# celo-org/celo-bls-snark-rs

Hardware: AMD Instinct MI355X
Metric: BLS12-377 G1 MSM scalar-muls/sec (higher is better)
Workload: dtype u32 limbs (28-bit radix, 64-bit column accumulators); 1 GPU; BLS12-377 G1 Pippenger MSM, 2^20 random bases/scalars per GPU, inputs resident in HBM; bases_per_gpu=1048576, window_bits=16, windows=16, buckets=524288

## Files before the change

celo-bls-snark-rs_amd/csrc/msm_engine.h:

```cpp
#pragma once

namespace celo {

extern "C" int celo_ifma_available();
extern "C" int celo_ifma_horner_377(const uint64_t* pts, size_t stride, const int32_t* order, int steps, uint64_t* out, int* inf);
extern "C" int celo_ifma_horner_761(const uint64_t* pts, size_t stride, const int32_t* order, int steps, uint64_t* out, int* inf);
typedef int (*ifma_horner_fn)(const uint64_t*, size_t, const int32_t*, int, uint64_t*, int*);
template <class F> struct IfmaHorner { static constexpr ifma_horner_fn fn = nullptr; };
template <> struct IfmaHorner<Fp<P377>> { static constexpr ifma_horner_fn fn = &celo_ifma_horner_377; };
template <> struct IfmaHorner<Fp<P761>> { static constexpr ifma_horner_fn fn = &celo_ifma_horner_761; };

struct MsmTimings {
  float convert = 0, sort = 0, accumulate = 0, reduce = 0, total = 0;
};

}
#include "msm_ba.h"
namespace celo {
template <> struct BaCfg<G_761> { static constexpr bool enabled = true; };

struct MsmTuning {
  bool narrow_windows, use_glv, use_gls, gls_force, lane_bitsum, host_threads, seg_occupancy, side_convert, side_convert_all, fx_compact;
  uint32_t seg_min, seg_min_shard, bitsum_lanes_max_shard;
  int seg_halves;
// ... 77 lines not shown
  bool host_threads = MsmTuning::get().host_threads;
  bool lane_horner = true;
  bool lane_bitsum = MsmTuning::get().lane_bitsum;
  uint32_t BITSUM_LANES_MAX = MsmTuning::get().bitsum_lanes_max;

  struct Plan { bool glv; uint32_t n; int sbits, c, nw, kn; };
  Plan plan(size_t n_) const {
    Plan p;
    p.glv = GlvExpand<G>::AVAILABLE && big_subgroup_points && use_glv && n_ >= (size_t(1) << 14);
    p.n = p.glv ? 2u * (uint32_t)n_ : (uint32_t)n_;
    p.sbits = p.glv ? GlvExpand<G>::BITS : G::SCALAR_BITS;
    p.c = force_c ? force_c : (p.glv ? window_bits_glv(p.n) : window_bits(p.n));
    p.nw = (p.sbits + p.c) / p.c;
    p.kn = narrow_top(p.c) ? p.nw * p.c - (p.sbits + 1) : 0;
    return p;
  }
  static int window_bit(const Plan& p, int w) {
    const int wide = p.nw - p.kn;
    return w < wide ? w * p.c : wide * p.c + (w - wide) * (p.c - 1);
  }
  int run_device(const uint64_t* d_ark_bases, const uint8_t* d_inf, const uint32_t* d_scalars, size_t n_, uint64_t* out_jac,
                 hipStream_t stream) {
    return run_device_windows(d_ark_bases, d_inf, d_scalars, n_, 0, 0, out_jac, nullptr, stream);
  }
  struct HostIn { const uint64_t* bases; const uint8_t* inf; const uint64_t* scalars; uint32_t chunks, head_split, tail_split; bool ark_zero; };
  static constexpr uint32_t HOST_HEAD_SPLIT_DEFAULT = 1, HOST_TAIL_SPLIT_DEFAULT = 0;
  int run_device_windows(const uint64_t* d_ark_bases, const uint8_t* d_inf, const uint32_t* d_scalars, size_t n_, int win_lo, int win_cnt,
                         uint64_t* out_jac, uint64_t* out_xyzz, hipStream_t stream, const FixedTable* fx = nullptr, const HostIn* hin = nullptr) {
    if (n_ == 0) {
      if (out_jac) write_identity(out_jac);
      if (out_xyzz) memset(out_xyzz, 0, 4 * IO::ARK64 * 8);
      return 0;
    }
    if (n_ >= (size_t(1) << 30)) return 2;
    if (fx && (win_cnt || n_ > fx->n || fx->cf < 16 || fx->cf > 22)) return 2;
    Plan pl = plan(n_);
    uint32_t fx_Ep = 0;
    uint8_t* d_fx_v8 = nullptr; uint16_t* d_fx_dg = nullptr; uint32_t* d_fx_cnt = nullptr;
    if (fx && fx->NV > 2 && fx->NV <= 128 && !win_cnt && n_ <= fx->n && fx->cf >= 16 && fx->cf <= 22 && MsmTuning::get().fx_compact) {
      const size_t E = fx->E();
      const size_t o_dg = (E + 255) & ~size_t(255), o_cnt = o_dg + ((E * 2 + 255) & ~size_t(255)), need = o_cnt + 256 * 4;
      if (need > fxs_bytes) {
        if (fxs) (void)hipFree(fxs);
        fxs = nullptr; fxs_bytes = 0;
        HIP_TRY(hipMalloc((void**)&fxs, need + need / 8), 1);
        fxs_bytes = need + need / 8;
      }
      d_fx_v8 = fxs; d_fx_dg = (uint16_t*)(fxs + o_dg); d_fx_cnt = (uint32_t*)(fxs + o_cnt);
      HIP_TRY(hipMemsetAsync(d_fx_cnt, 0, 256 * 4, stream), 1);
      hipLaunchKernelGGL((k_fixed_digits_c<SW, G::SCALAR_BITS>), dim3((fx->n + 255) / 256), dim3(256), 0, stream, d_scalars, fx->tinf, d_fx_v8, d_fx_dg, d_fx_cnt, fx->n,
                         (uint32_t)n_, fx->cf, fx->W, fx->NV, fx->M);
      uint32_t h_cnt[128];
      HIP_TRY(hipMemcpyAsync(h_cnt, d_fx_cnt, fx->NV * 4, hipMemcpyDeviceToHost, stream), 1);
      HIP_TRY(hipStreamSynchronize(stream), 1);
      uint32_t mx = 0;
      for (uint32_t v = 0; v < fx->NV; v++) mx = h_cnt[v] > mx ? h_cnt[v] : mx;
      const uint64_t ep = ((uint64_t)mx + 4095) & ~uint64_t(4095);
      if (ep >= 4096 && ep * 2 <= E) fx_Ep = (uint32_t)ep;
    }
    if (fx) { pl.glv = false; pl.n = fx_Ep ? fx_Ep : fx->E(); pl.sbits = G::SCALAR_BITS; pl.c = 16; pl.nw = (int)fx->NV; pl.kn = 0; }
    if (hin && (fx || pl.glv || win_cnt || hin->chunks < 1 || hin->chunks > 64 || !side_stream_.get() || !sort_stream_.get())) return 2;
    const bool glv = pl.glv;
    const uint32_t n = pl.n;
    const int sbits = pl.sbits, c = pl.c, nw_all = pl.nw;
    if (win_cnt < 0 || win_lo < 0 || (win_cnt && win_lo + win_cnt > nw_all)) return 2;
    const int w0 = win_cnt ? win_lo : 0;
    const int nw = win_cnt ? win_cnt : nw_all;
    if ((uint64_t)n * (uint64_t)nw_all >= (uint64_t(1) << 32)) return 2;
    const uint32_t B = 1u << (c - 1);
    const uint32_t total = (uint32_t)nw * B;
    uint32_t K = 0, cm = n;
    uint32_t clen[HOST_CHUNKS_MAX];
    if (hin) K = host_chunk_plan(n, hin->chunks, hin->head_split, hin->tail_split, cm, clen);
    const uint32_t ns = hin ? cm : n, nws = hin ? K * (uint32_t)nw : (uint32_t)nw, vw = hin ? (uint32_t)nw : 0u;
    const uint32_t npad = hin ? K * cm : n;
    if ((uint64_t)npad * (uint64_t)nw_all >= (uint64_t(1) << 32)) return 2;
    const uint32_t total_s = nws * B;
    const int seg_h = MsmTuning::get().seg_halves ? MsmTuning::get().seg_halves : (glv ? 3 : 4);
    uint32_t SEG = (uint32_t)seg_h * ((fx && !fx_Ep ? n / (uint32_t)nw_all : ns) / B + 1) / 2;
    uint32_t seg_min = MsmTuning::get().seg_min;
    if (win_cnt && MsmTuning::get().seg_occupancy) {
      const uint64_t adds = (uint64_t)n * (uint64_t)nw;
      const uint32_t lanes = (sizeof(F) <= 14 * sizeof(uint32_t)) ? 131072u : 65536u;
      const uint32_t occ = (uint32_t)((adds + lanes - 1) / lanes);
      if (occ < SEG) { SEG = occ; seg_min = MsmTuning::get().seg_min_shard; }
    }
    if (fx && !MsmTuning::get().seg_halves) {
      const uint32_t lanes = (sizeof(F) <= 14 * sizeof(uint32_t)) ? 131072u : 65536u;
      const uint32_t occ = fx->E() / (lanes * 8u) + 1u;
      if (occ < SEG) SEG = occ;
    }
    if (SEG < seg_min) SEG = seg_min;
    if (SEG > SIZE_BINS - 1) SEG = SIZE_BINS - 1;
    const uint32_t PW = B + ns / SEG + 1;
    const uint32_t slots = nws * PW;
    const int LB = c - 1;
    const uint32_t res_pts = (uint32_t)(LB + 1) * (uint32_t)nw;
    const uint32_t half_pts = (uint32_t)nw * (B / 2 + B / 4);

    size_t off = 0;
    auto take = [&](size_t bytes) { size_t o = off; off += (bytes + 255) & ~size_t(255); return o; };
    const size_t o_bases = take(fx ? 0 : (size_t)npad * IO::AFF_WORDS * 4);
    const size_t o_sc2 = take(glv ? (size_t)n * 16 : 0);
    const size_t o_digits = take((size_t)npad * nw_all * 2);
    const size_t o_remap = take(fx_Ep ? (size_t)n * nw_all * 4 : 0);
    const size_t o_sorted = take((size_t)ns * nws * 4);
    const uint32_t HIB = LB < 8 ? 0u : (uint32_t)LB - 8u, NBIN = 1u << HIB;
    uint32_t KB2 = ns / (64 * NBIN > 4096 ? 64 * NBIN : 4096);
    if (KB2 < 1) KB2 = 1;
    if (KB2 > 64) KB2 = 64;
    const uint32_t chunk2 = (ns + KB2 - 1) / KB2;
    const size_t o_blockcnt = take((size_t)nws * NBIN * KB2 * 4);
    const size_t o_binstart = take((size_t)nws * (NBIN + 1) * 4);
    const size_t o_tileprefix = take((size_t)nws * (NBIN + 1) * 4);
    const size_t o_recidx = take((size_t)ns * nws * 4);
    const size_t o_reckey = take((size_t)ns * nws);
    const size_t o_counts = take((size_t)total_s * 4);
    const size_t o_starts = take((size_t)total_s * 4);
    const size_t o_piecesof = take((size_t)total_s * 4);
    const size_t o_plen = take((size_t)slots * 4);
    constexpr size_t BINS_STRIDE = SIZE_BINS + 64;
    const size_t o_bins = take(BINS_STRIDE * 4 * (hin ? K : 1u));
    const size_t o_zero_end = off;
    const size_t o_pfirst = take((size_t)total_s * 4);
    const size_t o_big = take((size_t)total_s * 4);
    const size_t o_mid = take((size_t)total_s * 4);
    const size_t o_pbucket = take(hin ? (size_t)slots * 4 : 0);
    const size_t o_carrier = take(hin ? (size_t)total * IO::XYZZ_WORDS * 4 : 0);
    const size_t o_pstart = take((size_t)slots * 4);
    const size_t o_order = take((size_t)slots * 4);
    const size_t o_partials = take((size_t)slots * IO::XYZZ_WORDS * 4);
    const size_t o_work = take(((size_t)res_pts + 2 * (size_t)half_pts + 64) * IO::XYZZ_WORDS * 4);
    const int ba_ovr = batched_affine_override().load();
    const bool use_ba = BaCfg<G>::enabled && !hin && !fx && (ba_ovr >= 0 ? ba_ovr != 0 : MsmTuning::get().batched_affine != 0) && ns / B >= 8;
    const int ba_occ = MsmTuning::get().ba_occ;
    uint32_t ba_lanes = use_ba ? BA_LANES_OCC1 * (uint32_t)ba_occ * MsmTuning::get().ba_rounds : 0;
    if (use_ba && ba_lanes > (slots + 255) / 256 * 256) ba_lanes = (slots + 255) / 256 * 256;
    const uint32_t ba_pref_slots = use_ba ? ((slots + ba_lanes - 1) / ba_lanes) * (SEG / 2) : 0;
    const size_t o_ba_pts = take(use_ba ? (size_t)ns * nws * IO::AFF_WORDS * 4 : 0);
    const size_t o_ba_pref = take(use_ba ? (size_t)ba_pref_slots * ba_lanes * F::WORDS * 4 : 0);
    if (ensure(off)) return 1;
    if (res_pts > H_OUT_POINTS) return 2;
    char* A = arena;
    uint32_t* d_bases = fx ? fx->table : (uint32_t*)(A + o_bases);
    uint16_t* d_digits_all = (uint16_t*)(A + o_digits);
    uint16_t* d_digits = d_digits_all + (size_t)w0 * n;
    uint32_t* d_sorted = (uint32_t*)(A + o_sorted);
    uint32_t* d_blockcnt = (uint32_t*)(A + o_blockcnt);
    uint32_t* d_binstart = (uint32_t*)(A + o_binstart);
    uint32_t* d_recidx = (uint32_t*)(A + o_recidx);
    uint8_t* d_reckey = (uint8_t*)(A + o_reckey);
    uint32_t* d_tileprefix = (uint32_t*)(A + o_tileprefix);
    uint32_t* d_counts = (uint32_t*)(A + o_counts);
    uint32_t* d_starts = (uint32_t*)(A + o_starts);
    uint32_t* d_pfirst = (uint32_t*)(A + o_pfirst);
    uint32_t* d_piecesof = (uint32_t*)(A + o_piecesof);
    uint32_t* d_big = (uint32_t*)(A + o_big);
    uint32_t* d_mid = (uint32_t*)(A + o_mid);
    uint32_t* d_pstart = (uint32_t*)(A + o_pstart);
    uint32_t* d_plen = (uint32_t*)(A + o_plen);
    uint32_t* d_order = (uint32_t*)(A + o_order);
    uint32_t* d_bins = (uint32_t*)(A + o_bins);
    uint32_t* d_nwork = d_bins + SIZE_BINS;
    uint32_t* d_nbig = d_bins + SIZE_BINS + 1;
    uint32_t* d_nmid = d_bins + SIZE_BINS + 2;
    uint32_t* d_partials = (uint32_t*)(A + o_partials);
    uint32_t* d_work = (uint32_t*)(A + o_work);

    uint32_t* d_pbucket = hin ? (uint32_t*)(A + o_pbucket) : nullptr;
    uint32_t* d_carrier = hin ? (uint32_t*)(A + o_carrier) : nullptr;
    HIP_TRY(hipEventRecord(ev[0], stream), 1);
    const uint32_t region = ns / NBIN;
    const uint32_t ts_threads = region <= 2048 ? 256u : region <= 4096 ? 512u : 1024u;
    const uint32_t TILE = TILE_EPT * ts_threads, max_tiles = NBIN + ns / TILE + 1;
    uint32_t* d_remap = fx_Ep ? (uint32_t*)(A + o_remap) : nullptr;
    auto sort_windows = [&](uint32_t wb, uint32_t wn, hipStream_t st) {
      hipLaunchKernelGGL((k_part_hist<G>), dim3(KB2, wn), dim3(1024), 0, st, d_digits, d_blockcnt, ns, chunk2, NBIN, wb);
      hipLaunchKernelGGL((k_part_scan<G>), dim3(wn), dim3(1024), 0, st, d_blockcnt, d_binstart, d_tileprefix, NBIN, KB2, TILE, wb);
      hipLaunchKernelGGL((k_part_scatter<G>), dim3(KB2, wn), dim3(1024), 0, st, d_digits, d_blockcnt, d_recidx, d_reckey, ns, chunk2, HIB, NBIN, (const uint32_t*)d_remap, vw, wb);
      hipLaunchKernelGGL((k_tile_count<G>), dim3(max_tiles, wn), dim3(ts_threads), 0, st, d_reckey, d_binstart, d_tileprefix, d_counts, ns, B, HIB, NBIN, wb);
      hipLaunchKernelGGL((k_tile_sort<G>), dim3(max_tiles, wn), dim3(ts_threads), 0, st, d_recidx, d_reckey, d_binstart, d_tileprefix, d_counts,
                         d_starts, d_sorted, d_pfirst, d_pstart, d_plen, d_big, d_nbig, d_mid, d_nmid, ns, B, HIB, NBIN, SEG, PW, d_pbucket, vw, wb);
    };
    if (hin) {
      hipStream_t cs = side_stream_.get(), ss = sort_stream_.get();
      struct Drain { hipStream_t a, b, c; bool armed; ~Drain() { if (armed) { (void)hipStreamSynchronize(a); (void)hipStreamSynchronize(b); (void)hipStreamSynchronize(c); } } } drain{cs, ss, stream, true};
      if (ev_copy.size() < 3 * (size_t)K + 1) {
        const size_t have = ev_copy.size();
        ev_copy.resize(3 * (size_t)K + 1, nullptr);
        for (size_t i = have; i < ev_copy.size(); i++) HIP_TRY(hipEventCreateWithFlags(&ev_copy[i], hipEventDisableTiming), 1);
      }
      hipEvent_t* ev_sc = ev_copy.data();
      hipEvent_t* ev_bs = ev_copy.data() + K;
      hipEvent_t* ev_so = ev_copy.data() + 2 * K;
      HIP_TRY(hipMemsetAsync(d_counts, 0, o_zero_end - o_counts, stream), 1);
      HIP_TRY(hipMemsetAsync(d_carrier, 0, (size_t)total * IO::XYZZ_WORDS * 4, stream), 1);
      HIP_TRY(hipEventRecord(ev_copy[3 * K], stream), 1);
      HIP_TRY(hipStreamWaitEvent(ss, ev_copy[3 * K], 0), 1);
      constexpr size_t PT_BYTES = 2 * (size_t)IO::ARK64 * 8;
      const uint32_t cslots = (uint32_t)nw * PW;
      ArkCoord<IO::ARK64> ark_one;
      F::one().to_ark(ark_one.v);
      if (hin->ark_zero && d_inf != d_in_inf) return 2;
      size_t hlo = 0;
      for (uint32_t k = 0; k < K; hlo += clen[k], k++) {
        const size_t lo = (size_t)k * cm, cnt = clen[k];
        if (hin->ark_zero) {
          HIP_TRY(hipMemcpyAsync((char*)d_ark_bases + lo * PT_BYTES, (const char*)hin->bases + hlo * PT_BYTES, cnt * PT_BYTES, hipMemcpyHostToDevice, cs), 1);
          HIP_TRY(hipEventRecord(ev_bs[k], cs), 1);
        }
        HIP_TRY(hipMemcpyAsync((char*)d_scalars + lo * SW * 4, (const char*)hin->scalars + hlo * SW * 4, cnt * SW * 4, hipMemcpyHostToDevice, cs), 1);
        if (hin->inf) HIP_TRY(hipMemcpyAsync((char*)d_inf + lo, hin->inf + hlo, cnt, hipMemcpyHostToDevice, cs), 1);
        HIP_TRY(hipEventRecord(ev_sc[k], cs), 1);
        HIP_TRY(hipStreamWaitEvent(ss, ev_sc[k], 0), 1);
        if (hin->ark_zero) {
          HIP_TRY(hipStreamWaitEvent(ss, ev_bs[k], 0), 1);
          hipLaunchKernelGGL((k_flag_ark_zero<G>), dim3((unsigned)((cnt + 255) / 256)), dim3(256), 0, ss, d_ark_bases + lo * 2 * IO::ARK64,
                             hin->inf ? d_inf + lo : nullptr, d_in_inf + lo, cnt, ark_one);
        }
        if (launch_digits<SW, G::SCALAR_BITS>(c, d_scalars, d_inf, d_digits_all, (uint32_t)(lo + cnt), ss, cm, (k + 1) * cm, k * cm)) return 3;
        sort_windows(k * (uint32_t)nw, (uint32_t)nw, ss);
        uint32_t* bins_k = d_bins + (size_t)k * BINS_STRIDE;
        hipLaunchKernelGGL((k_size_hist<G>), dim3(cslots / 256 < 512 ? (cslots + 255) / 256 : 512), dim3(256), 0, ss, d_plen + (size_t)k * cslots, bins_k, cslots);
        hipLaunchKernelGGL((k_size_scan<G>), dim3(1), dim3(1024), 0, ss, bins_k, bins_k + SIZE_BINS);
        hipLaunchKernelGGL((k_size_scatter<G>), dim3((cslots + 4095) / 4096), dim3(1024), 0, ss, d_plen + (size_t)k * cslots, bins_k, d_order + (size_t)k * cslots, cslots);
        HIP_TRY(hipEventRecord(ev_so[k], ss), 1);
        if (k == 0) {
          HIP_TRY(hipStreamWaitEvent(stream, ev_so[0], 0), 1);
          HIP_TRY(hipEventRecord(ev[1], stream), 1);
          HIP_TRY(hipEventRecord(ev[2], stream), 1);
        }
        if (!hin->ark_zero) {
          HIP_TRY(hipMemcpyAsync((char*)d_ark_bases + lo * PT_BYTES, (const char*)hin->bases + hlo * PT_BYTES, cnt * PT_BYTES, hipMemcpyHostToDevice, cs), 1);
          HIP_TRY(hipEventRecord(ev_bs[k], cs), 1);
        }
        HIP_TRY(hipStreamWaitEvent(stream, ev_bs[k], 0), 1);
        if (k) HIP_TRY(hipStreamWaitEvent(stream, ev_so[k], 0), 1);
        hipLaunchKernelGGL((k_convert_bases<G>), dim3((unsigned)((cnt + 255) / 256)), dim3(256), 0, stream, d_ark_bases + lo * 2 * IO::ARK64, d_bases + lo * IO::AFF_WORDS, cnt);
        hipLaunchKernelGGL((k_accumulate_chunk<G>), dim3((cslots + 255) / 256), dim3(256), 0, stream, d_bases, d_sorted, d_pstart + (size_t)k * cslots, d_plen + (size_t)k * cslots,
                           d_order + (size_t)k * cslots, bins_k + SIZE_BINS, d_partials + (size_t)k * cslots * IO::XYZZ_WORDS, d_pbucket + (size_t)k * cslots, d_carrier, k ? 1u : 0u);
      }
      drain.armed = false;
    } else {
    const bool side = (win_cnt || MsmTuning::get().side_convert_all) && !glv && MsmTuning::get().side_convert && side_stream_.get() && ev_side[0];
    if (fx) {
    } else if (side) {
      HIP_TRY(hipEventRecord(ev_side[0], stream), 1);
      HIP_TRY(hipStreamWaitEvent(side_stream_.get(), ev_side[0], 0), 1);
      hipLaunchKernelGGL((k_convert_bases<G>), dim3((n + 255) / 256), dim3(256), 0, side_stream_.get(), d_ark_bases, d_bases, (size_t)n);
      HIP_TRY(hipEventRecord(ev_side[1], side_stream_.get()), 1);
    } else if (glv) GlvExpand<G>::launch(d_ark_bases, d_inf, d_scalars, (uint32_t)n_, d_bases, (uint32_t*)(A + o_sc2), stream);
    else hipLaunchKernelGGL((k_convert_bases<G>), dim3((n + 255) / 256), dim3(256), 0, stream, d_ark_bases, d_bases, (size_t)n);
    HIP_TRY(hipEventRecord(ev[1], stream), 1);
    if (fx && fx_Ep) {
      HIP_TRY(hipMemsetAsync(d_digits_all, 0xFF, (size_t)n * nw_all * 2, stream), 1);
      HIP_TRY(hipMemsetAsync(d_fx_cnt + 128, 0, 128 * 4, stream), 1);
      const uint32_t E32 = (uint32_t)fx->E();
      hipLaunchKernelGGL((k_fixed_place<G>), dim3((E32 + 1023) / 1024 < 4096 ? (E32 + 1023) / 1024 : 4096), dim3(1024), 0, stream, d_fx_v8, d_fx_dg, d_fx_cnt + 128, d_digits_all,
                         d_remap, E32, n, fx->NV);
    } else if (fx) hipLaunchKernelGGL((k_fixed_digits<SW, G::SCALAR_BITS>), dim3((fx->n + 255) / 256), dim3(256), 0, stream, d_scalars, fx->tinf, d_digits_all, fx->n, (uint32_t)n_,
                               fx->cf, fx->W, fx->NV, fx->M);
    else if (glv) { if (launch_digits<4, GlvExpand<G>::BITS>(c, (const uint32_t*)(A + o_sc2), nullptr, d_digits_all, n, stream)) return 3; }
    else if (launch_digits<SW, G::SCALAR_BITS>(c, d_scalars, d_inf, d_digits_all, n, stream)) return 3;
    HIP_TRY(hipMemsetAsync(d_counts, 0, o_zero_end - o_counts, stream), 1);
    sort_windows(0, (uint32_t)nw, stream);
    hipLaunchKernelGGL((k_size_hist<G>), dim3(slots / 256 < 512 ? (slots + 255) / 256 : 512), dim3(256), 0, stream, d_plen, d_bins, slots);
    hipLaunchKernelGGL((k_size_scan<G>), dim3(1), dim3(1024), 0, stream, d_bins, d_nwork);
    hipLaunchKernelGGL((k_size_scatter<G>), dim3((slots + 4095) / 4096), dim3(1024), 0, stream, d_plen, d_bins, d_order, slots);
    if (side) HIP_TRY(hipStreamWaitEvent(stream, ev_side[1], 0), 1);
    HIP_TRY(hipEventRecord(ev[2], stream), 1);
    if constexpr (BaCfg<G>::enabled) if (use_ba) {
      uint32_t* d_ba_pts = (uint32_t*)(A + o_ba_pts);
      const int levels = MsmTuning::get().ba_levels;
      if (ba_occ == 2)
        hipLaunchKernelGGL((k_ba_levels<G, 2>), dim3(ba_lanes / 256), dim3(256), 0, stream, d_bases, d_sorted, d_pstart, d_plen, d_order, d_nwork, d_ba_pts,
                           (uint32_t*)(A + o_ba_pref), ba_lanes, levels, ba_pref_slots);
      else
        hipLaunchKernelGGL((k_ba_levels<G, 1>), dim3(ba_lanes / 256), dim3(256), 0, stream, d_bases, d_sorted, d_pstart, d_plen, d_order, d_nwork, d_ba_pts,
                           (uint32_t*)(A + o_ba_pref), ba_lanes, levels, ba_pref_slots);
      hipLaunchKernelGGL((k_accumulate_ba<G>), dim3((slots + 255) / 256), dim3(256), 0, stream, d_ba_pts, d_pstart, d_plen, d_order, d_nwork, d_partials, levels);
    }
    if (!use_ba) launch_accumulate<G>(slots, stream, d_bases, d_sorted, d_pstart, d_plen, d_order, d_nwork, d_partials);
    }
    HIP_TRY(hipEventRecord(ev[3], stream), 1);
    const uint32_t mid_blocks = win_cnt ? (total + 20) / 21 < 16384 ? (total + 20) / 21 : 16384 : 1024;
    const uint32_t cfirst = hin ? 1u : 0u;
    if (lane_bitsum) hipLaunchKernelGGL((k_combine_mid_lanes<G>), dim3(mid_blocks), dim3(64), 0, stream, d_mid, d_nmid, d_counts, d_pfirst, d_partials, d_piecesof, SEG, cfirst);
    else hipLaunchKernelGGL((k_combine_mid<G>), dim3(256), dim3(128), 0, stream, d_mid, d_nmid, d_counts, d_pfirst, d_partials, d_piecesof, SEG, cfirst);
    hipLaunchKernelGGL((k_combine_big<G>), dim3(256), dim3(256), 0, stream, d_big, d_nbig, d_counts, d_pfirst, d_partials, d_piecesof, SEG, cfirst);
    const uint32_t* d_leaf = d_partials;
    const uint32_t* d_leaf_counts = d_counts;
    if (hin) {
      hipLaunchKernelGGL((k_merge_carried<G>), dim3((total + 127) / 128), dim3(128), 0, stream, d_counts, d_pfirst, d_partials, d_carrier, total, K, SEG);
      d_leaf = d_carrier; d_leaf_counts = nullptr;
    }
    {
      struct Arr { uint32_t at, per_window; bool born; int level; };
      uint32_t half_at[2] = {res_pts, res_pts + half_pts};
      Arr tree = {0, B, true, LB};
      std::vector<Arr> lists;
      for (int t = 1; t <= LB; t++) {
        BitsumJobs jobs;
        jobs.njobs = 0;
        uint32_t cursor = half_at[t & 1], total_out = 0;
        auto push = [&](uint32_t src, uint32_t outs_per_window, uint32_t mode, int result_slot) -> uint32_t {
          const uint32_t outs = outs_per_window * (uint32_t)nw;
          uint32_t dst;
          if (result_slot >= 0) dst = (uint32_t)result_slot * (uint32_t)nw;
          else { dst = cursor; cursor += outs; }
          const int j = (int)jobs.njobs++;
          total_out += outs;
          jobs.end[j] = total_out; jobs.src[j] = src; jobs.dst[j] = dst; jobs.mode[j] = mode;
          return dst;
        };
        std::vector<Arr> next_lists;
        if (tree.level >= 2) {
          const uint32_t outs = tree.per_window / 4;
          const uint32_t dst = push(tree.at, outs, tree.level == LB ? 3u : 1u, outs == 1 ? tree.level : -1);
          if (outs > 1) next_lists.push_back({dst, outs, false, tree.level});
        } else {
          push(tree.at, 1, 4u, 1);
        }
        for (const Arr& L : lists) {
          const uint32_t outs = L.per_window / 2;
          const uint32_t dst = push(L.at, outs, 0u, outs == 1 ? L.level : -1);
          if (outs > 1) next_lists.push_back({dst, outs, false, L.level});
        }
        {
          const uint32_t outs = tree.per_window / 2;
          const uint32_t dst = push(tree.at, outs, tree.level == LB ? 2u : 0u, outs == 1 ? 0 : -1);
          tree = {dst, outs, true, tree.level - 1};
        }
        lists.swap(next_lists);
        if (lane_bitsum && total_out <= (win_cnt ? MsmTuning::get().bitsum_lanes_max_shard : BITSUM_LANES_MAX))
          hipLaunchKernelGGL((k_bitsum_lanes<G>), dim3((total_out + 20) / 21), dim3(64), 0, stream, d_leaf, d_leaf_counts, d_pfirst, d_piecesof, SEG, d_work, jobs);
        else
          hipLaunchKernelGGL((k_bitsum<G>), dim3((total_out + 127) / 128), dim3(128), 0, stream, d_leaf, d_leaf_counts, d_pfirst, d_piecesof, SEG,
                             d_work, jobs);
      }
      hipLaunchKernelGGL((k_results_to_ark<G>), dim3((4 * res_pts + 63) / 64), dim3(64), 0, stream, d_work, res_pts);
    }
    HIP_TRY(hipEventRecord(ev[4], stream), 1);
    HIP_TRY(hipMemcpyAsync(h_out, d_work, (size_t)res_pts * IO::XYZZ_WORDS * 4, hipMemcpyDeviceToHost, stream), 1);
    HIP_TRY(hipEventRecord(ev[5], stream), 1);
    HIP_TRY(hipStreamSynchronize(stream), 1);
    HIP_TRY(hipGetLastError(), 1);
    (void)hipEventElapsedTime(&tm.convert, ev[0], ev[1]);
    (void)hipEventElapsedTime(&tm.sort, ev[1], ev[2]);
    (void)hipEventElapsedTime(&tm.accumulate, ev[2], ev[3]);
    (void)hipEventElapsedTime(&tm.reduce, ev[3], ev[4]);
    (void)hipEventElapsedTime(&tm.total, ev[0], ev[5]);
    last_c = c; last_nw = nw; last_buckets = total; last_glv = glv;
    typedef typename HostField<F>::type HF;
    const uint64_t* h64 = reinterpret_cast<const uint64_t*>(h_out);
    constexpr size_t PT64 = (size_t)IO::XYZZ_WORDS / 2;
    horner_steps.clear();
    const int kn = pl.kn;
    (void)sbits;
    if (fx) {
      int top = LB - 1;
      while (((uint64_t)(nw - 1) * fx->M) >> (top + 1)) top++;
      for (int t = top; t >= 0; t--) {
        horner_steps.push_back(-1);
        for (int v = 0; v < nw; v++) if ((((uint64_t)v * fx->M) >> t) & 1) horner_steps.push_back(v | HORNER_NODBL);
        if (t <= LB - 1) for (int v = 0; v < nw; v++) horner_steps.push_back(((LB - t) * nw + v) | HORNER_NODBL);
      }
      for (int v = 0; v < nw; v++) horner_steps.push_back(v | HORNER_NODBL);
    } else
    for (int w = nw - 1; w >= 0; w--) {
      horner_steps.push_back(-1);
      for (int l = (w0 + w >= nw_all - kn ? 2 : 1); l <= LB; l++) horner_steps.push_back(l * nw + w);
      horner_steps.push_back(w | HORNER_NODBL);
    }
    auto run_list = [&](const int32_t* steps, int count) {
      if (IfmaHorner<F>::fn && celo_ifma_available()) {
        uint64_t r[4 * IO::ARK64];
        int inf = 0;
        if (IfmaHorner<F>::fn(h64, PT64, steps, count, r, &inf) == 0) return inf ? HXyzz<HF>::identity() : HXyzz<HF>::load(r, IO::ARK64);
      }
      return host64_horner<HF>(h64, PT64, IO::ARK64, steps, count);
    };
    constexpr int HT = (sizeof(HF) > 6 * 8) ? HOST_HORNER_THREADS : 1;
    HXyzz<HF> total_pt;
    if (HT > 1 && host_threads && (fx ? horner_steps.size() >= 64 : nw >= 2 * HT)) {
      int start[HT + 1], dbls[HT];
      if (fx) {
        int adds_total = 0;
        for (int k = 0; k < (int)horner_steps.size(); k++) adds_total += horner_steps[k] >= 0 ? 1 : 0;
        int g = 0, adds = 0;
        start[0] = 0;
        for (int k = 0; k < (int)horner_steps.size(); k++) {
          if (horner_steps[k] < 0 && g + 1 < HT && k > start[g] && adds * HT >= (g + 1) * adds_total) start[++g] = k;
          adds += horner_steps[k] >= 0 ? 1 : 0;
        }
        while (g + 1 < HT) start[++g] = (int)horner_steps.size();
        start[HT] = (int)horner_steps.size();
        for (int j = 0; j < HT; j++) {
          dbls[j] = 0;
          for (int k = start[j]; k < start[j + 1]; k++) if (horner_steps[k] < 0 || !(horner_steps[k] & HORNER_NODBL)) dbls[j]++;
        }
      } else {
        int wdone = 0, g = 0;
        start[0] = 0;
        for (int k = 0; k < (int)horner_steps.size(); k++) {
          if (horner_steps[k] >= 0 && (horner_steps[k] & HORNER_NODBL)) {
            wdone++;
            if (wdone == (g + 1) * nw / HT && g + 1 < HT) start[++g] = k + 1;
          }
        }
        start[HT] = (int)horner_steps.size();
        for (int j = 0; j < HT; j++) {
          dbls[j] = 0;
          for (int k = start[j]; k < start[j + 1]; k++) if (horner_steps[k] < 0 || !(horner_steps[k] & HORNER_NODBL)) dbls[j]++;
        }
      }
      HXyzz<HF> part[HT];
      std::thread th[HT - 1];
      bool started[HT - 1];
      for (int j = 1; j < HT; j++) {
        started[j - 1] = true;
        try { th[j - 1] = std::thread([&, j] { part[j] = run_list(horner_steps.data() + start[j], start[j + 1] - start[j]); }); }
        catch (const std::system_error&) { started[j - 1] = false; }
      }
      part[0] = run_list(horner_steps.data() + start[0], start[1] - start[0]);
      for (int j = 1; j < HT; j++) {
        if (started[j - 1]) th[j - 1].join();
        else part[j] = run_list(horner_steps.data() + start[j], start[j + 1] - start[j]);
      }
      total_pt = part[0];
      for (int j = 1; j < HT; j++) {
        for (int d = 0; d < dbls[j]; d++) total_pt = hxyzz_dbl(total_pt);
        hxyzz_add(total_pt, part[j]);
      }
    } else {
      total_pt = run_list(horner_steps.data(), (int)horner_steps.size());
    }
    if (out_xyzz) {
      if (total_pt.is_identity()) memset(out_xyzz, 0, 4 * IO::ARK64 * 8);
      else { total_pt.X.store(out_xyzz); total_pt.Y.store(out_xyzz + IO::ARK64); total_pt.ZZ.store(out_xyzz + 2 * IO::ARK64); total_pt.ZZZ.store(out_xyzz + 3 * IO::ARK64); }
    }
    if (out_jac) write_host_jacobian(total_pt, out_jac);
    return 0;
  }
  typedef typename HostField<F>::type HostF;
  static void write_host_jacobian(const HXyzz<HostF>& pt, uint64_t* out_jac) {
    if (pt.is_identity()) { write_identity(out_jac); return; }
    (pt.X * pt.ZZ).store(out_jac);
    (pt.Y * pt.ZZZ).store(out_jac + IO::ARK64);
    pt.ZZ.store(out_jac + 2 * IO::ARK64);
  }

  int run_host(const uint64_t* bases, const uint8_t* inf, const uint64_t* scalars, size_t n, uint64_t* out_jac, hipStream_t stream) {
    return run_host_windows(bases, inf, scalars, n, 0, 0, out_jac, nullptr, stream);
  }
  int run_host_windows(const uint64_t* bases, const uint8_t* inf, const uint64_t* scalars, size_t n, int win_lo, int win_cnt, uint64_t* out_jac,
                       uint64_t* out_xyzz, hipStream_t stream) {
    if (n == 0) return run_device_windows(nullptr, nullptr, nullptr, 0, win_lo, win_cnt, out_jac, out_xyzz, stream);
    const int ovr = host_chunks_override().load();
    const bool fq2_group = sizeof(F) > 14 * sizeof(uint32_t) && G::SCALAR_BITS <= 256;
    uint32_t by_size = (uint32_t)(n >> (fq2_group ? 19 : 18));
    const uint32_t lo_k = G::SCALAR_BITS > 256 ? 8u : 4u, hi_k = fq2_group ? 8u : 16u;
    by_size = by_size < lo_k ? lo_k : by_size > hi_k ? hi_k : by_size;
    uint32_t chunks = ovr >= 0 ? (uint32_t)(ovr & 0xFF) : MsmTuning::get().host_chunks != 0xFFFFFFFFu ? MsmTuning::get().host_chunks : by_size;
    uint32_t head_split = ovr >= 0 && ((ovr >> 8) & 15) ? (uint32_t)((ovr >> 8) & 15) - 1u : MsmTuning::get().host_head_split != 0xFFFFFFFFu ? MsmTuning::get().host_head_split : HOST_HEAD_SPLIT_DEFAULT;
    uint32_t tail_split = ovr >= 0 && ((ovr >> 12) & 15) ? (uint32_t)((ovr >> 12) & 15) - 1u : MsmTuning::get().host_tail_split != 0xFFFFFFFFu ? MsmTuning::get().host_tail_split : HOST_TAIL_SPLIT_DEFAULT;
    if (chunks > 64) chunks = 64;
    const size_t min_chunk_log = ovr >= 0 ? 16 : 17;
    if (chunks > (n >> min_chunk_log)) chunks = (uint32_t)(n >> min_chunk_log);
    const bool glv_plan = plan(n).glv;
    const bool glv_off = glv_plan && !ark_zero_identity && !win_cnt && n >= (size_t(1) << 19);
    if (!(ovr >= 0 && ((ovr >> 8) & 15)) && MsmTuning::get().host_head_split == 0xFFFFFFFFu && chunks && n / chunks < (size_t(1) << 18)) head_split = 0;
    bool pipelined = chunks >= (ovr >= 0 ? 1u : 2u) && !win_cnt && (!glv_plan || glv_off) && n < (size_t(1) << 30) && (!ark_zero_identity || ovr >= 0 || n >= (size_t(1) << 21));
    size_t need = n;
    if (pipelined) {
      uint32_t cm, clen[HOST_CHUNKS_MAX];
      need = (size_t)host_chunk_plan(n, chunks, head_split, tail_split, cm, clen) * cm;
      uint64_t nw_run;
      { struct GlvOff { bool& f; bool was; GlvOff(bool& x, bool off) : f(x), was(x) { if (off) f = false; } ~GlvOff() { f = was; } } g(use_glv, glv_plan);
        nw_run = (uint64_t)plan(n).nw; }
      if ((uint64_t)need * nw_run >= (uint64_t(1) << 32)) { pipelined = false; need = n; }
    }
    const size_t n_real = n;
    n = need;
    if (n > cap_in) {
      if (d_in_bases) (void)hipFree(d_in_bases);
      if (d_in_scalars) (void)hipFree(d_in_scalars);
      if (d_in_inf) (void)hipFree(d_in_inf);
      d_in_bases = nullptr; d_in_scalars = nullptr; d_in_inf = nullptr; cap_in = 0;
      HIP_TRY(hipMalloc(&d_in_bases, n * 2 * IO::ARK64 * 8), 1);
      HIP_TRY(hipMalloc(&d_in_scalars, n * SW * 4), 1);
      HIP_TRY(hipMalloc(&d_in_inf, n), 1);
      cap_in = n;
    }
    n = n_real;
    if (pipelined) {
      const HostIn hin = {bases, inf, scalars, chunks, head_split, tail_split, ark_zero_identity};
      struct GlvOff { bool& f; bool was; GlvOff(bool& x, bool off) : f(x), was(x) { if (off) f = false; } ~GlvOff() { f = was; } } glv_guard(use_glv, glv_plan);
      return run_device_windows(d_in_bases, inf || ark_zero_identity ? d_in_inf : nullptr, (const uint32_t*)d_in_scalars, n, 0, 0, out_jac, out_xyzz, stream, nullptr, &hin);
    }
    HIP_TRY(hipMemcpyAsync(d_in_bases, bases, n * 2 * IO::ARK64 * 8, hipMemcpyHostToDevice, stream), 1);
    HIP_TRY(hipMemcpyAsync(d_in_scalars, scalars, n * SW * 4, hipMemcpyHostToDevice, stream), 1);
    if (inf) HIP_TRY(hipMemcpyAsync(d_in_inf, inf, n, hipMemcpyHostToDevice, stream), 1);
    if (ark_zero_identity) {
      ArkCoord<IO::ARK64> one;
      F::one().to_ark(one.v);
      hipLaunchKernelGGL((k_flag_ark_zero<G>), dim3((unsigned)((n + 255) / 256)), dim3(256), 0, stream, d_in_bases, inf ? d_in_inf : nullptr, d_in_inf, n, one);
      return run_device_windows(d_in_bases, d_in_inf, (const uint32_t*)d_in_scalars, n, win_lo, win_cnt, out_jac, out_xyzz, stream);
    }
    return run_device_windows(d_in_bases, inf ? d_in_inf : nullptr, (const uint32_t*)d_in_scalars, n, win_lo, win_cnt, out_jac, out_xyzz, stream);
  }

  int run_fixed(const FixedTable& T, const void* scalars, size_t n_sc, int resident, uint64_t* out_jac, hipStream_t stream) {
    if (n_sc > T.n) n_sc = T.n;
    if (n_sc == 0) { write_identity(out_jac); return 0; }
    const uint32_t* d_sc = (const uint32_t*)scalars;
    if (!resident) {
      if (n_sc > cap_fx) {
        if (d_fx_scalars) (void)hipFree(d_fx_scalars);
        d_fx_scalars = nullptr; cap_fx = 0;
        HIP_TRY(hipMalloc(&d_fx_scalars, n_sc * SW * 4), 1);
        cap_fx = n_sc;
      }
      HIP_TRY(hipMemcpyAsync(d_fx_scalars, scalars, n_sc * SW * 4, hipMemcpyHostToDevice, stream), 1);
      d_sc = (const uint32_t*)d_fx_scalars;
    }
    return run_device_windows(nullptr, nullptr, d_sc, n_sc, 0, 0, out_jac, nullptr, stream, &T);
  }
  static int fixed_window_bits(size_t n) {
    int lg = 0;
    while ((size_t(1) << lg) < n * ((G::SCALAR_BITS + 16) / 16)) lg++;
    int cf = lg - 4;
    const int top = sizeof(F) > 14 * sizeof(uint32_t) ? 21 : 20;
    return cf < 16 ? 16 : cf > top ? top : cf;
  }
  static int fixed_build(const uint64_t* d_ark_bases, const uint8_t* d_inf, size_t n_, int cf, FixedTable* T, hipStream_t stream) {
    if (n_ == 0 || n_ >= (size_t(1) << 27)) return 2;
    auto fits = [&](int c_) {
      const uint64_t W_ = (uint64_t)((G::SCALAR_BITS + c_) / c_), M_ = c_ == 16 ? 32768u : 32767u, NV_ = ((uint64_t(1) << (c_ - 1)) - 1u) / M_ + 1u;
      return (uint64_t)n_ * W_ < (uint64_t(1) << 31) && (uint64_t)n_ * W_ * NV_ < (uint64_t(1) << 32);
    };
    if (cf == 0) {
      cf = fixed_window_bits(n_);
      while (cf > 16 && !fits(cf)) cf--;
    }
    if (cf < 16 || cf > 22 || !fits(cf)) return 2;
    const uint32_t n = (uint32_t)n_, W = (uint32_t)((G::SCALAR_BITS + cf) / cf);
    const uint32_t M = cf == 16 ? 32768u : 32767u, NV = ((1u << (cf - 1)) - 1u) / M + 1u;
    const size_t E = (size_t)n * W;
    hipEvent_t e0 = nullptr, e1 = nullptr;
    HIP_TRY(hipEventCreate(&e0), 1); HIP_TRY(hipEventCreate(&e1), 1);
    T->n = n; T->W = W; T->NV = NV; T->M = M; T->cf = cf; T->device = api_device();
    T->bytes = E * IO::AFF_WORDS * 4 + E;
    HIP_TRY(hipMalloc(&T->table, E * IO::AFF_WORDS * 4), 1);
    HIP_TRY(hipMalloc(&T->tinf, E), 1);
    HIP_TRY(hipEventRecord(e0, stream), 1);
    hipLaunchKernelGGL((k_convert_bases<G>), dim3((n + 255) / 256), dim3(256), 0, stream, d_ark_bases, T->table, (size_t)n);
    hipLaunchKernelGGL((k_fixed_first_flags<G>), dim3((n + 255) / 256), dim3(256), 0, stream, d_inf, T->tinf, n);
    for (uint32_t j = 1; j < W; j++)
      hipLaunchKernelGGL((k_fixed_next<G>), dim3((n + 127) / 128), dim3(128), 0, stream, T->table + (size_t)(j - 1) * n * IO::AFF_WORDS, T->tinf + (size_t)(j - 1) * n,
                         T->table + (size_t)j * n * IO::AFF_WORDS, T->tinf + (size_t)j * n, n, cf);
    HIP_TRY(hipEventRecord(e1, stream), 1);
    HIP_TRY(hipStreamSynchronize(stream), 1);
    HIP_TRY(hipGetLastError(), 1);
    (void)hipEventElapsedTime(&T->build_ms, e0, e1);
    (void)hipEventDestroy(e0); (void)hipEventDestroy(e1);
    return 0;
  }

  static constexpr uint32_t BATCH_MAX_N = 1024;
  MsmTimings tm_batch;
  int batch_bits = 0;
  int bits_hint = 0, measured_bits = 0;
  int run_batch_host(const uint64_t* bases, const uint8_t* inf, const uint64_t* scalars, const uint32_t* offsets, size_t m,
                     uint64_t* out, hipStream_t stream) {
    return run_batch(bases, inf, scalars, 0, offsets, m, out, nullptr, stream);
  }
  int run_batch(const uint64_t* bases, const uint8_t* inf, const uint64_t* scalars, int resident, const uint32_t* offsets, size_t m,
                uint64_t* out, uint64_t** d_out_ret, hipStream_t stream) {
    measured_bits = 0;
    if (m == 0) return 0;
    const uint32_t total_pts = offsets[m];
    uint32_t max_n = 0;
    for (size_t p = 0; p < m; p++) {
      uint32_t k = offsets[p + 1] - offsets[p];
      if (k > max_n) max_n = k;
    }
    if (max_n > BATCH_MAX_N || total_pts == 0) {
      std::vector<uint64_t> hres;
      uint64_t* dst = out;
      if (!out) { hres.resize(m * 3 * IO::ARK64); dst = hres.data(); }
      for (size_t p = 0; p < m; p++) {
        const uint32_t lo = offsets[p], k = offsets[p + 1] - lo;
        const uint8_t* pi = inf ? inf + lo : nullptr;
        const int rc = resident ? run_device(bases + (size_t)lo * 2 * IO::ARK64, pi, (const uint32_t*)scalars + (size_t)lo * SW, k, dst + p * 3 * IO::ARK64, stream)
                                : run_host(bases + (size_t)lo * 2 * IO::ARK64, pi, scalars + (size_t)lo * (SW / 2), k, dst + p * 3 * IO::ARK64, stream);
        if (rc) return rc;
      }
      tm_batch = tm;
      if (!out) {
        const size_t bytes = m * 3 * IO::ARK64 * 8;
        if (bytes > side_out_bytes) {
          if (d_side_out) (void)hipFree(d_side_out);
          d_side_out = nullptr; side_out_bytes = 0;
          HIP_TRY(hipMalloc(&d_side_out, bytes), 1);
          side_out_bytes = bytes;
        }
// ... 263 lines not shown
```

celo-bls-snark-rs_amd/csrc/msm_reduce.h:

```cpp
#pragma once

namespace celo {

template <class G>
__global__ void __launch_bounds__(128) k_combine_mid(const uint32_t* __restrict__ mid, const uint32_t* __restrict__ nmid,
                                                     const uint32_t* __restrict__ counts, const uint32_t* __restrict__ pfirst,
                                                     uint32_t* __restrict__ partials, uint32_t* __restrict__ pieces_of, uint32_t SEG, uint32_t first = 0) {
  typedef typename G::F F;
  typedef PointIO<F> IO;
  for (uint32_t q = blockIdx.x * blockDim.x + threadIdx.x; q < *nmid; q += gridDim.x * blockDim.x) {
    uint32_t t = mid[q];
    uint32_t pc = (counts[t] + SEG - 1) / SEG - first, pf = pfirst[t] + first;
    Xyzz<F> acc = IO::load_xyzz(partials + (size_t)pf * IO::XYZZ_WORDS);
    for (uint32_t k = 1; k < pc; k++) {
      Xyzz<F> v = IO::load_xyzz(partials + (size_t)(pf + k) * IO::XYZZ_WORDS);
      xyzz_add_fn(acc, v);
    }
    IO::store_xyzz(partials + (size_t)pf * IO::XYZZ_WORDS, acc);
    pieces_of[t] = 1;
  }
}
template <class G>
__global__ void __launch_bounds__(64) k_combine_mid_lanes(const uint32_t* __restrict__ mid, const uint32_t* __restrict__ nmid,
                                                          const uint32_t* __restrict__ counts, const uint32_t* __restrict__ pfirst,
                                                          uint32_t* __restrict__ partials, uint32_t* __restrict__ pieces_of, uint32_t SEG, uint32_t first = 0) {
  typedef typename G::F F;
  typedef PointIO<F> IO;
  typedef QTriT<FieldBase<F>> QB;
  typedef LanePoint<QB> LP;
  const int g = QB::group();
  if (g >= 21) return;
  for (uint32_t q = blockIdx.x * 21u + (uint32_t)g; q < *nmid; q += gridDim.x * 21u) {
    const uint32_t t = mid[q];
    const uint32_t pc = (counts[t] + SEG - 1) / SEG - first, pf = pfirst[t] + first;
    const Xyzz<F> a = IO::load_xyzz(partials + (size_t)pf * IO::XYZZ_WORDS);
    typename LP::Pt acc = {{a.X, a.Y, a.ZZ, a.ZZZ}, a.is_identity()};
    for (uint32_t k = 1; k < pc; k++) {
      const Xyzz<F> v = IO::load_xyzz(partials + (size_t)(pf + k) * IO::XYZZ_WORDS);
      const typename LP::P pb = {v.X, v.Y, v.ZZ, v.ZZZ};
      LP::add(acc, pb, v.is_identity());
    }
    if (QB::lane() == 0) {
      const Xyzz<F> r = acc.inf ? Xyzz<F>::identity() : Xyzz<F>{acc.p.X, acc.p.Y, acc.p.ZZ, acc.p.ZZZ};
      IO::store_xyzz(partials + (size_t)pf * IO::XYZZ_WORDS, r);
      pieces_of[t] = 1;
    }
  }
}

template <class G>
__global__ void __launch_bounds__(256) k_combine_big(const uint32_t* __restrict__ big, const uint32_t* __restrict__ nbig,
                                                     const uint32_t* __restrict__ counts, const uint32_t* __restrict__ pfirst,
                                                     uint32_t* __restrict__ partials, uint32_t* __restrict__ pieces_of, uint32_t SEG, uint32_t first = 0) {
  typedef typename G::F F;
  typedef PointIO<F> IO;
  __shared__ uint32_t stage[64 * IO::XYZZ_WORDS];
  for (uint32_t q = blockIdx.x; q < *nbig; q += gridDim.x) {
    uint32_t t = big[q];
    uint32_t pc = (counts[t] + SEG - 1) / SEG - first, pf = pfirst[t] + first;
    Xyzz<F> acc = Xyzz<F>::identity();
    for (uint32_t k = threadIdx.x; k < pc; k += 256) {
      Xyzz<F> v = IO::load_xyzz(partials + (size_t)(pf + k) * IO::XYZZ_WORDS);
      xyzz_add_fn(acc, v);
    }
    for (uint32_t width = 256; width > 1; width >>= 2) {
      uint32_t q4 = width >> 2;
      for (uint32_t r = 1; r < 4; r++) {
        __syncthreads();
        if (threadIdx.x >= r * q4 && threadIdx.x < (r + 1) * q4) IO::store_xyzz(stage + (threadIdx.x - r * q4) * IO::XYZZ_WORDS, acc);
        __syncthreads();
        if (threadIdx.x < q4) { Xyzz<F> v = IO::load_xyzz(stage + threadIdx.x * IO::XYZZ_WORDS); xyzz_add_fn(acc, v); }
      }
    }
    __syncthreads();
    if (threadIdx.x == 0) { IO::store_xyzz(partials + (size_t)pf * IO::XYZZ_WORDS, acc); pieces_of[t] = 1; }
    __syncthreads();
  }
}

template <class G> HD Xyzz<typename G::F> load_bucket(const uint32_t* partials, const uint32_t* counts, const uint32_t* pfirst,
                                                       const uint32_t* pieces_of, uint32_t t, uint32_t SEG) {
  typedef typename G::F F;
  typedef PointIO<F> IO;
  if (!counts) return IO::load_xyzz(partials + (size_t)t * IO::XYZZ_WORDS);
  uint32_t c = counts[t];
  if (c == 0) return Xyzz<F>::identity();
  (void)pieces_of; (void)SEG;
  return IO::load_xyzz(partials + (size_t)pfirst[t] * IO::XYZZ_WORDS);
}

struct BitsumJobs {
  static constexpr int MAXJ = 20;
  uint32_t njobs;
  uint32_t end[MAXJ];
  uint32_t src[MAXJ];
  uint32_t dst[MAXJ];
  uint32_t mode[MAXJ];
};
template <class G>
__global__ void __launch_bounds__(128) k_bitsum(const uint32_t* __restrict__ partials, const uint32_t* __restrict__ counts,
                                                const uint32_t* __restrict__ pfirst, const uint32_t* __restrict__ pieces_of, uint32_t SEG,
                                                uint32_t* __restrict__ work, BitsumJobs jobs) {
  typedef typename G::F F;
  typedef PointIO<F> IO;
  const uint32_t t = blockIdx.x * blockDim.x + threadIdx.x;
  if (t >= jobs.end[jobs.njobs - 1]) return;
  uint32_t j = 0;
  while (t >= jobs.end[j]) j++;
  const uint32_t i = t - (j ? jobs.end[j - 1] : 0u);
  const uint32_t mode = jobs.mode[j];
  Xyzz<F> a, b;
  if (mode == 2) {
    a = load_bucket<G>(partials, counts, pfirst, pieces_of, 2 * i, SEG);
    b = load_bucket<G>(partials, counts, pfirst, pieces_of, 2 * i + 1, SEG);
  } else if (mode == 3) {
    a = load_bucket<G>(partials, counts, pfirst, pieces_of, 4 * i + 1, SEG);
    b = load_bucket<G>(partials, counts, pfirst, pieces_of, 4 * i + 3, SEG);
  } else {
    const uint32_t* in = work + (size_t)jobs.src[j] * IO::XYZZ_WORDS;
    const size_t ia = mode == 0 ? 2 * (size_t)i : mode == 1 ? 4 * (size_t)i + 1 : 2 * (size_t)i + 1;
    a = IO::load_xyzz(in + ia * IO::XYZZ_WORDS);
    if (mode != 4) b = IO::load_xyzz(in + (ia + (mode == 0 ? 1 : 2)) * IO::XYZZ_WORDS);
  }
  if (mode != 4) xyzz_add(a, b);
  IO::store_xyzz(work + ((size_t)jobs.dst[j] + i) * IO::XYZZ_WORDS, a);
}
template <class G>
__global__ void __launch_bounds__(64) k_bitsum_lanes(const uint32_t* __restrict__ partials, const uint32_t* __restrict__ counts,
                                                     const uint32_t* __restrict__ pfirst, const uint32_t* __restrict__ pieces_of, uint32_t SEG,
                                                     uint32_t* __restrict__ work, BitsumJobs jobs) {
  typedef typename G::F F;
  typedef PointIO<F> IO;
  typedef QTriT<FieldBase<F>> QB;
  typedef LanePoint<QB> LP;
  const int g = QB::group();
  const uint32_t t = blockIdx.x * 21u + (uint32_t)g;
  if (g >= 21 || t >= jobs.end[jobs.njobs - 1]) return;
  uint32_t j = 0;
  while (t >= jobs.end[j]) j++;
  const uint32_t i = t - (j ? jobs.end[j - 1] : 0u);
  const uint32_t mode = jobs.mode[j];
  Xyzz<F> a, b = Xyzz<F>::identity();
  if (mode == 2) {
    a = load_bucket<G>(partials, counts, pfirst, pieces_of, 2 * i, SEG);
    b = load_bucket<G>(partials, counts, pfirst, pieces_of, 2 * i + 1, SEG);
  } else if (mode == 3) {
    a = load_bucket<G>(partials, counts, pfirst, pieces_of, 4 * i + 1, SEG);
    b = load_bucket<G>(partials, counts, pfirst, pieces_of, 4 * i + 3, SEG);
  } else {
    const uint32_t* in = work + (size_t)jobs.src[j] * IO::XYZZ_WORDS;
    const size_t ia = mode == 0 ? 2 * (size_t)i : mode == 1 ? 4 * (size_t)i + 1 : 2 * (size_t)i + 1;
    a = IO::load_xyzz(in + ia * IO::XYZZ_WORDS);
    if (mode != 4) b = IO::load_xyzz(in + (ia + (mode == 0 ? 1 : 2)) * IO::XYZZ_WORDS);
  }
  typename LP::Pt acc = {{a.X, a.Y, a.ZZ, a.ZZZ}, a.is_identity()};
  if (mode != 4) {
    const typename LP::P pb = {b.X, b.Y, b.ZZ, b.ZZZ};
    LP::add(acc, pb, b.is_identity());
  }
  if (QB::lane() != 0) return;
  const Xyzz<F> r = acc.inf ? Xyzz<F>::identity() : Xyzz<F>{acc.p.X, acc.p.Y, acc.p.ZZ, acc.p.ZZZ};
  IO::store_xyzz(work + ((size_t)jobs.dst[j] + i) * IO::XYZZ_WORDS, r);
}
template <class G>
__global__ void __launch_bounds__(64) k_results_to_ark(uint32_t* __restrict__ work, uint32_t res_pts) {
  typedef typename G::F F;
  typedef PointIO<F> IO;
  const uint32_t t = blockIdx.x * blockDim.x + threadIdx.x, pt = t >> 2, q = t & 3;
  const bool live = pt < res_pts;
  uint64_t out[IO::ARK64];
  if (live) F::load(work + (size_t)pt * IO::XYZZ_WORDS + q * IO::FW).to_ark(out);
  __syncthreads();
  if (live) {
    uint64_t* o = reinterpret_cast<uint64_t*>(work + (size_t)pt * IO::XYZZ_WORDS) + q * IO::ARK64;
#pragma unroll
    for (int i = 0; i < IO::ARK64; i++) o[i] = out[i];
  }
}

}
```

Before: 333.5 million scalar-muls/s.

## Store bitsum tree work points in even/odd-split structure-of-arrays rows

Bitsum intermediate points beyond the result slots are now stored in a transposed layout. Each 16-byte vector of a point goes into its own row, and even and odd point indices are split into separate halves. Adjacent threads loading pair operands (2i, 2i+1) then read consecutive uint4s, which should coalesce the tree reduction's global loads and stores. It adds index arithmetic and assumes the np sizing covers every work slot; the bitsum tree is a small part of MSM time.

```diff
diff --git a/celo-bls-snark-rs_amd/csrc/msm_engine.h b/celo-bls-snark-rs_amd/csrc/msm_engine.h
--- a/celo-bls-snark-rs_amd/csrc/msm_engine.h
+++ b/celo-bls-snark-rs_amd/csrc/msm_engine.h
@@ -403,6 +403,7 @@
       for (int t = 1; t <= LB; t++) {
         BitsumJobs jobs;
         jobs.njobs = 0;
+        jobs.res_pts = res_pts; jobs.np = 2 * half_pts + 64;
         uint32_t cursor = half_at[t & 1], total_out = 0;
         auto push = [&](uint32_t src, uint32_t outs_per_window, uint32_t mode, int result_slot) -> uint32_t {
           const uint32_t outs = outs_per_window * (uint32_t)nw;
diff --git a/celo-bls-snark-rs_amd/csrc/msm_reduce.h b/celo-bls-snark-rs_amd/csrc/msm_reduce.h
--- a/celo-bls-snark-rs_amd/csrc/msm_reduce.h
+++ b/celo-bls-snark-rs_amd/csrc/msm_reduce.h
@@ -96,7 +96,30 @@
   uint32_t src[MAXJ];
   uint32_t dst[MAXJ];
   uint32_t mode[MAXJ];
+  uint32_t res_pts, np;
 };
+template <class F> struct WorkRows {
+  typedef PointIO<F> IO;
+  static constexpr int V = IO::XYZZ_WORDS / 4;
+  HD static size_t at(int v, uint32_t np, uint32_t p) { return (((size_t)(2 * v) + (p & 1u)) * (np >> 1) + (p >> 1)) * 4; }
+  HD static Xyzz<F> load(const uint32_t* rows, uint32_t np, uint32_t p) {
+    alignas(16) uint32_t w[IO::XYZZ_WORDS];
+#pragma unroll
+    for (int v = 0; v < V; v++) *reinterpret_cast<uint4*>(w + 4 * v) = *reinterpret_cast<const uint4*>(rows + at(v, np, p));
+    return IO::load_xyzz(w);
+  }
+  HD static void store(uint32_t* rows, uint32_t np, uint32_t p, const Xyzz<F>& a) {
+    alignas(16) uint32_t w[IO::XYZZ_WORDS];
+    IO::store_xyzz(w, a);
+#pragma unroll
+    for (int v = 0; v < V; v++) *reinterpret_cast<uint4*>(rows + at(v, np, p)) = *reinterpret_cast<const uint4*>(w + 4 * v);
+  }
+};
+template <class F> HD void store_work(uint32_t* work, const BitsumJobs& jobs, uint32_t at, const Xyzz<F>& a) {
+  typedef PointIO<F> IO;
+  if (at < jobs.res_pts) IO::store_xyzz(work + (size_t)at * IO::XYZZ_WORDS, a);
+  else WorkRows<F>::store(work + (size_t)jobs.res_pts * IO::XYZZ_WORDS, jobs.np, at - jobs.res_pts, a);
+}
 template <class G>
 __global__ void __launch_bounds__(128) k_bitsum(const uint32_t* __restrict__ partials, const uint32_t* __restrict__ counts,
                                                 const uint32_t* __restrict__ pfirst, const uint32_t* __restrict__ pieces_of, uint32_t SEG,
@@ -117,13 +140,13 @@
     a = load_bucket<G>(partials, counts, pfirst, pieces_of, 4 * i + 1, SEG);
     b = load_bucket<G>(partials, counts, pfirst, pieces_of, 4 * i + 3, SEG);
   } else {
-    const uint32_t* in = work + (size_t)jobs.src[j] * IO::XYZZ_WORDS;
-    const size_t ia = mode == 0 ? 2 * (size_t)i : mode == 1 ? 4 * (size_t)i + 1 : 2 * (size_t)i + 1;
-    a = IO::load_xyzz(in + ia * IO::XYZZ_WORDS);
-    if (mode != 4) b = IO::load_xyzz(in + (ia + (mode == 0 ? 1 : 2)) * IO::XYZZ_WORDS);
+    const uint32_t* rows = work + (size_t)jobs.res_pts * IO::XYZZ_WORDS;
+    const uint32_t ia = jobs.src[j] - jobs.res_pts + (mode == 0 ? 2 * i : mode == 1 ? 4 * i + 1 : 2 * i + 1);
+    a = WorkRows<F>::load(rows, jobs.np, ia);
+    if (mode != 4) b = WorkRows<F>::load(rows, jobs.np, ia + (mode == 0 ? 1 : 2));
   }
   if (mode != 4) xyzz_add(a, b);
-  IO::store_xyzz(work + ((size_t)jobs.dst[j] + i) * IO::XYZZ_WORDS, a);
+  store_work<F>(work, jobs, jobs.dst[j] + i, a);
 }
 template <class G>
 __global__ void __launch_bounds__(64) k_bitsum_lanes(const uint32_t* __restrict__ partials, const uint32_t* __restrict__ counts,
@@ -148,10 +171,10 @@
     a = load_bucket<G>(partials, counts, pfirst, pieces_of, 4 * i + 1, SEG);
     b = load_bucket<G>(partials, counts, pfirst, pieces_of, 4 * i + 3, SEG);
   } else {
-    const uint32_t* in = work + (size_t)jobs.src[j] * IO::XYZZ_WORDS;
-    const size_t ia = mode == 0 ? 2 * (size_t)i : mode == 1 ? 4 * (size_t)i + 1 : 2 * (size_t)i + 1;
-    a = IO::load_xyzz(in + ia * IO::XYZZ_WORDS);
-    if (mode != 4) b = IO::load_xyzz(in + (ia + (mode == 0 ? 1 : 2)) * IO::XYZZ_WORDS);
+    const uint32_t* rows = work + (size_t)jobs.res_pts * IO::XYZZ_WORDS;
+    const uint32_t ia = jobs.src[j] - jobs.res_pts + (mode == 0 ? 2 * i : mode == 1 ? 4 * i + 1 : 2 * i + 1);
+    a = WorkRows<F>::load(rows, jobs.np, ia);
+    if (mode != 4) b = WorkRows<F>::load(rows, jobs.np, ia + (mode == 0 ? 1 : 2));
   }
   typename LP::Pt acc = {{a.X, a.Y, a.ZZ, a.ZZZ}, a.is_identity()};
   if (mode != 4) {
@@ -160,7 +183,7 @@
   }
   if (QB::lane() != 0) return;
   const Xyzz<F> r = acc.inf ? Xyzz<F>::identity() : Xyzz<F>{acc.p.X, acc.p.Y, acc.p.ZZ, acc.p.ZZZ};
-  IO::store_xyzz(work + ((size_t)jobs.dst[j] + i) * IO::XYZZ_WORDS, r);
+  store_work<F>(work, jobs, jobs.dst[j] + i, r);
 }
 template <class G>
 __global__ void __launch_bounds__(64) k_results_to_ark(uint32_t* __restrict__ work, uint32_t res_pts) {
```

Result: no change. 334.7 million scalar-muls/s (median of 5 runs) (+0.3%).
